# Pixel-Talk/CanonSwap

Hardware: AMD Instinct MI355X
Metric: frames/sec at 512x512 (generator hot path F->W->T->R->W->G) (higher is better)
Workload: dtype f16; 1 GPU; BASELINE configs[2]: 512x512 video, 64 frames batched per launch on each GPU, steady state over 1280 frames (20 launches per GPU) (256x256 crops in, random-init weights of the real architecture); frames_per_launch_per_gpu=64, frames_total=1280, parallelism=frame-shard x1, identities_resident=1, latency_mode=False, accumulate=fp32, debug_decodes=False

## Files before the change

canonswap_amd/_isa.py:

```python
from __future__ import annotations

import os
import subprocess

from ._build import HALO_NGROUPS, OBJ_DIR


def _disassemble(obj_dir: str, objdump: str, oname: str) -> str:
    obj = os.path.join(obj_dir, oname)
    subprocess.run([objdump, "--offloading", obj], check=True, capture_output=True)
    co = obj + ".0.hipv4-amdgcn-amd-amdhsa--gfx950"
    try:
        return subprocess.run([objdump, "-d", "--no-show-raw-insn", co], check=True, capture_output=True, text=True).stdout
    finally:
        for f in os.listdir(obj_dir):
            if f.startswith(oname + ".0."):
                os.remove(os.path.join(obj_dir, f))


def isa_check(obj_dir: str | None = None) -> dict:
    import re
    obj_dir = obj_dir or OBJ_DIR
    objdump = os.environ.get("LLVM_OBJDUMP", "/opt/rocm/lib/llvm/bin/llvm-objdump")
    if not os.path.exists(objdump):
        raise FileNotFoundError(f"isa_check: {objdump} not found")
    seen = dict(_isa_check_wide(obj_dir, objdump))
    seen.update(_isa_check_lat(obj_dir, objdump))
    for g in range(HALO_NGROUPS):
        txt = _disassemble(obj_dir, objdump, f"conv_halo_g{g}.o")
        for m in re.finditer(r"^[0-9a-f]+ <(_Z16conv_halo_kernelILi\d+ELi\d+ELi(\d+)ELi\d+ELi\d+ELi\d+ELb[01]ELb[01]ELi0EEv10ConvParams)>:\n(.*?)(?=^[0-9a-f]+ <|\Z)",
                             txt, re.S | re.M):
            name, wch, body = m.group(1), int(m.group(2)), m.group(3).split("\n")
            want = f"s_waitcnt vmcnt({3 * wch})"
            kend = max(i for i, l in enumerate(body) if "v_mfma" in l)
            waits = [i for i, l in enumerate(body) if i < kend and l.strip().startswith(want) and "lgkmcnt" not in l]
            if len(waits) < 4:
                raise RuntimeError(f"isa_check: {name}: {len(waits)} x `{want}` in the K loop, expected 4 (one per ring slot)")
            waits = waits[:4]
            loads = [(i, re.search(r"global_load_dwordx4 v\[(\d+):(\d+)\], v\[\d+:\d+\], off", l)) for i, l in enumerate(body)]
            loads = [(i, int(q.group(1))) for i, q in loads if q]
            prime = [r for i, r in loads if i < waits[0]][-4 * wch:]
            if len(prime) != 4 * wch:
                raise RuntimeError(f"isa_check: {name}: the prologue primes {len(prime)} ring registers, expected {4 * wch}")
            for k, w in enumerate(waits):
                slot = prime[k * wch:(k + 1) * wch]
                end = waits[k + 1] if k + 1 < 4 else len(body)
                seg = body[w:end]
                rel = [i for i, r in loads if w < i < end and r in slot]
                if len(rel) < wch:
                    raise RuntimeError(f"isa_check: {name}: ring slot {k} is not reloaded into v{slot} after its wait")
                first_reload = min(rel) - w
                uses = [j for j, l in enumerate(seg[:first_reload]) if "v_mfma" in l and any(f"v[{r}:{r + 3}]" in l for r in slot)]
                if not uses:
                    raise RuntimeError(f"isa_check: {name}: no MFMA reads ring slot {k} (v{slot}) between its wait and its reload")
            tail = "\n".join(body[waits[-1]:])
            if "s_waitcnt vmcnt(0)" not in tail:
                raise RuntimeError(f"isa_check: {name}: the ring is not drained (s_waitcnt vmcnt(0)) before the epilogue")
            seen[name] = len(waits)
    if not seen:
        raise RuntimeError("isa_check: no dynamic-shape conv_halo kernel found in the objects (name mangling changed?)")
    return seen


def _isa_check_lat(obj_dir: str, objdump: str) -> dict:
    import re
    txt = _disassemble(obj_dir, objdump, "conv_lat.o")
    seen = {}
    for m in re.finditer(r"^[0-9a-f]+ <(\S*conv_lat_kernel\S*)>:\n(.*?)(?=^[0-9a-f]+ <|\Z)", txt, re.S | re.M):
        name, body = m.group(1), [l.split("//")[0].strip() for l in m.group(2).split("\n")]
        body = [l for l in body if l]
        mf = [i for i, l in enumerate(body) if l.startswith("v_mfma")]
        if not mf:
            raise RuntimeError(f"isa_check: {name}: no MFMA")
        if any(l.startswith(("s_cbranch", "s_branch")) for l in body[mf[0]:mf[-1]]):
            raise RuntimeError(f"isa_check: {name}: a branch inside the K loop (the walk assumes straight-line code)")
        for i, l in enumerate(body):
            if re.search(r"\bm0\b", l):
                ok = l.startswith("s_mov_b32 m0,") and any(b.startswith("buffer_load") and b.endswith("lds") for b in body[i + 1:i + 3])
                if not ok:
                    raise RuntimeError(f"isa_check: {name}: `{l}` touches m0 outside the hidden LDS-DMA sequence")
        nvm, open_dma, nbar, ndma = 0, [], 0, 0
        for i, l in enumerate(body[:mf[-1] + 1]):
            op = l.split()[0]
            if op.startswith(("global_load", "buffer_load", "global_store", "buffer_store", "scratch_load", "scratch_store")):
                if op.startswith("buffer_load") and l.endswith("lds"):
                    open_dma.append(nvm); ndma += 1
                nvm += 1
            if op == "s_barrier":
                nbar += 1
                w = next((body[j] for j in range(i - 1, max(i - 6, -1), -1) if body[j].startswith("s_waitcnt") and "vmcnt" in body[j]), None)
                if w is None and not open_dma:
                    continue
                if w is None:
                    raise RuntimeError(f"isa_check: {name}: barrier {nbar} of the K loop has no vmcnt wait in front of it")
                n = int(re.search(r"vmcnt\((\d+)\)", w).group(1))
                for idx in open_dma:
                    if nvm - idx - 1 < n:
                        raise RuntimeError(f"isa_check: {name}: `{w}` before barrier {nbar} does not cover a DMA piece issued {nvm - idx - 1} vector-memory instructions earlier")
                open_dma = []
        if open_dma:
            raise RuntimeError(f"isa_check: {name}: {len(open_dma)} DMA pieces are never waited for at a chunk head")
        if len(mf) not in (8 * 6 * 8, 8 * 6 * 16) or ndma != 24:
            raise RuntimeError(f"isa_check: {name}: {len(mf)} MFMAs / {ndma} DMA instructions, expected 384 or 768 / 24")
        seen[name] = len(mf)
    if not seen:
        raise RuntimeError("isa_check: no conv_lat kernel found in conv_lat.o (name mangling changed?)")
    return seen


def _isa_check_wide(obj_dir: str, objdump: str) -> dict:
    seen = _isa_check_ring(obj_dir, objdump, "conv_wide.o", r"\S*conv_wide_kernel\S*", 18 * 64)
    seen.update(_isa_check_ring(obj_dir, objdump, "conv_halo_g1.o", r"_Z16conv_halo_kernelILi32ELi8ELi5ELi2ELi2ELi0ELb1ELb0ELi[789]E\S*", None))
    return seen
# ... 67 lines not shown
```

canonswap_amd/csrc/common.h:

```cpp
#pragma once
#include <hip/hip_runtime.h>
#include <stdint.h>

typedef _Float16 half_t;
typedef _Float16 h8_t __attribute__((ext_vector_type(8)));
typedef _Float16 h4_t __attribute__((ext_vector_type(4)));
typedef float f4_t __attribute__((ext_vector_type(4)));

enum { ACT_NONE = 0, ACT_RELU = 1, ACT_LRELU = 2, ACT_SIGMOID = 3, ACT_GELU = 4 };
enum { MODE_STD = 0, MODE_TBLEND = 1, MODE_SPADE = 2, MODE_PIXSHUF = 3,
       MODE_STDSTAT = 4 };
enum { CFG_128x128 = 0, CFG_128x64 = 1, CFG_256x32 = 2, CFG_256x16 = 3 };
enum { CFG_H_128x128 = 10, CFG_H_128x64 = 11, CFG_H_256x32 = 12, CFG_H_128x32 = 13, CFG_H_128x16 = 14, CFG_H_256x16 = 15,
       CFG_H_SK128x32 = 16 , CFG_H_128x256 = 17,
       CFG_H_128x160 = 18 ,
       CFG_H_256x160 = 19 ,
       CFG_H_256x64 = 20 ,
       CFG_VOL32 = 30 , CFG_WIDE = 31 ,
       CFG_LAT = 32  };

struct TDesc {
    void* p;
    long sN, sD, sH, sW;
};

struct ConvParams {
    const half_t* in;
    const half_t* zero;
    long in_sN, in_sD, in_sH, in_sW;
    int N, D, H, W;
    int inD;
    int Cin;
    int cg, cg_cin;
    long in_sG;
    int nchunks;
    int up_shift;
    int KD, KH, KW, PD, PH, PW;
    const half_t* wgt;
    const long* wofs;
    const int* wslot;
    int Cout_pad;
    int Cout;
    int lgTW, lgTH, lgTD;
    int nTW, nTH, nTD, nTN;
    const float* bias;
    const float* bias2;
    int act0;
    float slope0;
    TDesc res;
    int res_f32;
    int res_shift;
    const float* pixscale;
    int ps_stride;
    TDesc out0;
    int out0_f32;
    const float* s2;
    const float* t2;
    int act1;
    float slope1;
    TDesc out1;
    const float* stats;
    float* stat_out;
    float* sk_out;
    int sk_splits;
    int ragged;
    unsigned mg_ncb, mg_tw, mg_th, mg_td;
    int hilo;
    int xcd_map;
    float* kw_out;
    int ep_general;
// ... 216 lines not shown
```

canonswap_amd/csrc/conv_halo.hip:

```cpp
#include "conv_halo_kernel.h"

#ifndef HALO_GROUP
#define HALO_GROUP (-1)
#endif
#define IN_GROUP(g) (HALO_GROUP == -1 || HALO_GROUP == (g))
#define NOT_MINE (-2)

template <int CK, int WPX, int WCH, int WVP, int WVC, int MODE, bool SK, int STV>
static int launch_halo_cfg(const ConvParams& p, hipStream_t st)
{
    if constexpr (STV != 0) {
        using SS = StaticShape<STV>;
        if (p.KD == SS::KD && p.KH == SS::KH && p.KW == SS::KW && p.lgTW == SS::LW && p.lgTH == SS::LH && p.lgTD == SS::LD &&
            p.nchunks % (CK / 32) == 0)
            return launch_halo_st<CK, WPX, WCH, WVP, WVC, MODE, SK, STV>(p, st);
    }
    if constexpr (WCH == 4 && MODE == MODE_STDSTAT) {
        cs_set_error("conv_halo: the 128x256 statistics tile exists for the static shapes only (%dx%dx%d taps, tile 2^%d x 2^%d x 2^%d)",
                     p.KD, p.KH, p.KW, p.lgTW, p.lgTH, p.lgTD);
        return -1;
    } else {
        return launch_halo_st<CK, WPX, WCH, WVP, WVC, MODE, SK, 0>(p, st);
    }
}

#define HALO_CASE(CFG, WPX, WCH, WVP, WVC, MODE, SK, ST2D, ST3D)                                         \
    if (cfg == CFG && mode == MODE) {                                                                    \
        if (ck == 64) return launch_halo_cfg<64, WPX, WCH, WVP, WVC, MODE, SK, ST2D>(p, st);            \
        if (stv == 1) return launch_halo_cfg<32, WPX, WCH, WVP, WVC, MODE, SK, ST2D>(p, st);            \
        if (stv == 5 && ST3D == 2) return launch_halo_cfg<32, WPX, WCH, WVP, WVC, MODE, SK, (ST3D == 2 ? 5 : 0)>(p, st); \
        return launch_halo_cfg<32, WPX, WCH, WVP, WVC, MODE, SK, ST3D>(p, st);                           \
    }

#define GROUP_FN(g) int launch_conv_halo_g##g(const ConvParams& p, int cfg, int ck, int mode, int stv, hipStream_t st)
GROUP_FN(0); GROUP_FN(1); GROUP_FN(2); GROUP_FN(3); GROUP_FN(4); GROUP_FN(5); GROUP_FN(6); GROUP_FN(7);

#if IN_GROUP(0)
GROUP_FN(0)
{
    (void)stv;
    if (p.KD == 3 && p.KH == 2 && p.KW == 2 && ck == 32 && mode == MODE_STD) {
        if (cfg == CFG_H_256x32) return launch_halo_cfg<32, 4, 2, 4, 1, MODE_STD, false, 12>(p, st);
        if (cfg == CFG_H_128x64) return launch_halo_cfg<32, 4, 2, 2, 2, MODE_STD, false, 13>(p, st);
        if (cfg == CFG_H_128x128 && p.lgTW == 2) return launch_halo_cfg<32, 8, 2, 1, 4, MODE_STD, false, 17>(p, st);
        if (cfg == CFG_H_128x128) return launch_halo_cfg<32, 8, 2, 1, 4, MODE_STD, false, 13>(p, st);
    }
    if (mode == MODE_STD && p.KD == 1 && p.KH == 1 && p.KW == 1) {
        if (cfg == CFG_H_128x128 && ck == 32) return launch_halo_cfg<32, 8, 2, 1, 4, MODE_STD, false, 15>(p, st);
        if (cfg == CFG_H_128x64 && ck == 64) return launch_halo_cfg<64, 4, 2, 2, 2, MODE_STD, false, 15>(p, st);
        if (cfg == CFG_H_128x64 && ck == 32) return launch_halo_cfg<32, 4, 2, 2, 2, MODE_STD, false, 15>(p, st);
        if (cfg == CFG_H_128x32 && ck == 64) return launch_halo_cfg<64, 2, 2, 4, 1, MODE_STD, false, 15>(p, st);
        if (cfg == CFG_H_128x32 && ck == 32) return launch_halo_cfg<32, 2, 2, 4, 1, MODE_STD, false, 15>(p, st);
    }
    return NOT_MINE;
}
#endif

#if IN_GROUP(1)
GROUP_FN(1)
{
    if (cfg == CFG_H_128x128 && mode == MODE_STD && ck == 64 && p.KD == 1 && p.KH <= 2 && p.KW <= 2) {
        if (p.KH == 2 && p.KW == 2) return launch_halo_cfg<64, 8, 2, 1, 4, MODE_STD, false, 10>(p, st);
        if (p.KH == 2) return launch_halo_cfg<64, 8, 2, 1, 4, MODE_STD, false, 11>(p, st);
        if (p.KW == 2) return launch_halo_cfg<64, 8, 2, 1, 4, MODE_STD, false, 14>(p, st);
        return launch_halo_cfg<64, 8, 2, 1, 4, MODE_STD, false, 15>(p, st);
    }
    if (cfg == CFG_H_256x64 && mode == MODE_STD && ck == 32) return launch_halo_cfg<32, 8, 2, 2, 2, MODE_STD, false, 7>(p, st);
    if (cfg == CFG_H_256x64 && ck == 64) {
        if (p.KD != 1 || p.KH != 3 || p.KW != 3 || p.lgTW != 4 || p.lgTH != 4 || p.lgTD != 0) {
            cs_set_error("conv_halo: the 2-D 256x64 tile runs 3x3 convs on 16x16 tiles only");
            return -1;
        }
        if (mode == MODE_STD) return launch_halo_st<64, 8, 2, 2, 2, MODE_STD, false, 16>(p, st);
        if (mode == MODE_STDSTAT) return launch_halo_st<64, 8, 2, 2, 2, MODE_STDSTAT, false, 16>(p, st);
    }
    if (cfg == CFG_H_256x160 && mode == MODE_STD && ck == 32) {
        if (p.KD == 7 && p.lgTW == 2) return launch_halo_cfg<32, 8, 5, 2, 2, MODE_STD, false, 9>(p, st);
        if (p.KD == 7) return launch_halo_cfg<32, 8, 5, 2, 2, MODE_STD, false, 8>(p, st);
        return launch_halo_cfg<32, 8, 5, 2, 2, MODE_STD, false, 7>(p, st);
    }
    if (cfg == CFG_H_128x160 && mode == MODE_STD && ck == 32) {
        if (stv == 4) return launch_halo_cfg<32, 4, 5, 2, 2, MODE_STD, false, 4>(p, st);
        if (stv == 6) return launch_halo_cfg<32, 4, 5, 2, 2, MODE_STD, false, 6>(p, st);
        return launch_halo_cfg<32, 4, 5, 2, 2, MODE_STD, false, 2>(p, st);
    }
    return NOT_MINE;
}
#endif

#if IN_GROUP(2)
GROUP_FN(2)
{
    HALO_CASE(CFG_H_128x256, 8, 4, 1, 4, MODE_STD, false, 1, 0)
    HALO_CASE(CFG_H_128x256, 8, 4, 1, 4, MODE_TBLEND, false, 1, 0)
// ... 73 lines not shown
```

canonswap_amd/csrc/conv_halo_kernel.h:

```cpp
#pragma once
#include <type_traits>
#include <utility>
#include <cstdlib>
#include "common.h"
#ifdef CS_TIMELINE
#define EP_TL(i) TL_STAMP(i)
#endif
#define EP_POOL_WSH_V EP_POOL_WSH_K
#define EP_POOL_HSH_V EP_POOL_HSH_K
#define EP_SPMUL_V EP_SPMUL_K
#define EP_DUP_V EP_DUP_K
#define EP_MLIN_V EP_MLIN_K
#define EP_O1ONLY_V EP_O1ONLY_K
#define EP_O0_EXTRA_V ep_o0_extra
#include "conv_epilogue.h"

typedef unsigned int u4_t __attribute__((ext_vector_type(4)));
__device__ __forceinline__ unsigned mdiv(unsigned u, unsigned magic) { return magic ? __umulhi(u, magic) : u; }

template <int OFF>
__device__ __forceinline__ void wfrag_load(u4_t& dst, const half_t* ptr)
{
    asm volatile("global_load_dwordx4 %0, %1, off offset:%2" : "=v"(dst) : "v"(ptr), "n"(OFF));
}
template <int N>
__device__ __forceinline__ void wait_vmcnt_le()
{
    asm volatile("s_waitcnt vmcnt(%0)" ::"n"(N) : "memory");
}

#ifdef CS_TIMELINE
extern unsigned long long* g_cs_tl;
extern long g_cs_tl_cap;
#define TL_STAMP(i) do { __builtin_amdgcn_sched_barrier(0); tl_t[i] = __builtin_amdgcn_s_memtime(); __builtin_amdgcn_sched_barrier(0); } while (0)
#else
#define TL_STAMP(i) do { } while (0)
#endif

template <int ST> struct StaticShape { static constexpr int KD = 0, KH = 0, KW = 0, LW = 0, LH = 0, LD = 0; };
template <> struct StaticShape<1> { static constexpr int KD = 1, KH = 3, KW = 3, LW = 4, LH = 3, LD = 0; };
template <> struct StaticShape<2> { static constexpr int KD = 3, KH = 3, KW = 3, LW = 3, LH = 3, LD = 1; };
template <> struct StaticShape<3> { static constexpr int KD = 3, KH = 3, KW = 3, LW = 2, LH = 2, LD = 4; };
template <> struct StaticShape<4> { static constexpr int KD = 7, KH = 7, KW = 1, LW = 3, LH = 3, LD = 1; };
template <> struct StaticShape<5> { static constexpr int KD = 3, KH = 3, KW = 3, LW = 2, LH = 2, LD = 3; };
template <> struct StaticShape<6> { static constexpr int KD = 7, KH = 7, KW = 1, LW = 1, LH = 3, LD = 3; };
template <> struct StaticShape<7> { static constexpr int KD = 3, KH = 3, KW = 3, LW = 3, LH = 3, LD = 2; };
template <> struct StaticShape<8> { static constexpr int KD = 7, KH = 7, KW = 1, LW = 1, LH = 3, LD = 4; };
template <> struct StaticShape<9> { static constexpr int KD = 7, KH = 7, KW = 1, LW = 2, LH = 3, LD = 3; };
template <> struct StaticShape<16> { static constexpr int KD = 1, KH = 3, KW = 3, LW = 4, LH = 4, LD = 0; };
template <> struct StaticShape<12> { static constexpr int KD = 3, KH = 2, KW = 2, LW = 2, LH = 2, LD = 4; };
template <> struct StaticShape<13> { static constexpr int KD = 3, KH = 2, KW = 2, LW = 3, LH = 3, LD = 1; };
template <> struct StaticShape<17> { static constexpr int KD = 3, KH = 2, KW = 2, LW = 2, LH = 2, LD = 3; };
template <> struct StaticShape<10> { static constexpr int KD = 1, KH = 2, KW = 2, LW = 4, LH = 3, LD = 0; };
template <> struct StaticShape<11> { static constexpr int KD = 1, KH = 2, KW = 1, LW = 4, LH = 3, LD = 0; };
template <> struct StaticShape<14> { static constexpr int KD = 1, KH = 1, KW = 2, LW = 4, LH = 3, LD = 0; };
template <> struct StaticShape<15> { static constexpr int KD = 1, KH = 1, KW = 1, LW = 4, LH = 3, LD = 0; };

template <int CK, int WPX, int WCH, int WVP, int ST, int MODE> constexpr int halo_pad()
{
    if (CK == 64 && WCH == 4 && WPX == 8 && ST == 1) return 2;
    if (CK == 32 && WCH == 5 && WPX == 8 && (ST == 7 || ST == 8 || ST == 9)) return 2;
    if (CK == 64 && WCH == 2 && WPX == 8 && WVP == 2 && ST == 16) return 2;
    if (CK == 32 && WCH == 2 && WPX == 8 && ST == 1 && MODE == MODE_SPADE) return 2;
    return 1;
}
template <int ST, int PAD> constexpr int halo_hi()
{
    if (PAD == 2) return ST == 3 ? 16 : (ST == 9 ? 19 : ((ST == 7 || ST == 8) ? 15 : (ST == 16 ? 13 : 8)));
    return ST == 4 ? 18 : ((ST == 3 || ST == 7 || ST == 8 || ST == 9) ? 13 : (ST == 12 ? 9 : 8));
}
template <int ST, int PAD> __host__ __device__ constexpr int halo_lane_pos(int l)
{
    using SS = StaticShape<ST>;
    if (ST == 0 || SS::KW != 3 || SS::LW > 3 || SS::LW < 2) return l;
    if (SS::LW == 2 && PAD == 2) return ((l & 1) << 1) | ((l & 2) << 2) | ((l >> 2) & 1) | ((l & 8) >> 1);
    return ((l & 1) << 1) | ((l & 2) << 1) | ((l >> 2) & 1) | (l & 8);
}

template <class F, int... I> __device__ __forceinline__ void halo_static_for_impl(F&& f, std::integer_sequence<int, I...>) { (f(std::integral_constant<int, I>{}), ...); }
template <int N, class F> __device__ __forceinline__ void halo_static_for(F&& f) { halo_static_for_impl(static_cast<F&&>(f), std::make_integer_sequence<int, N>{}); }

template <int WCH, int PFS, int HI, int ST0>
constexpr int halo_ring_young(int st, int L, int NP, bool dma_cur)
{
    auto dma = [&](int u, bool on) { return (on && u >= ST0 && u < ST0 + HI) ? 1 : 0; };
    auto cur_before = [&](int from_step ) {
        int n = 0;
        for (int u = from_step; u < st; ++u) n += (u >= 1 ? WCH : 0) + dma(u, dma_cur);
        return n;
    };
    if (st >= PFS) {
        const int u0 = st - PFS + 1;
        return dma(u0, dma_cur) + cur_before(u0 + 1);
    }
    const int prime = (PFS - 1 - st) * WCH + cur_before(0);
    int g = 0;
    if (NP % PFS == 0) g = st + NP - PFS + 1;
    else { for (int u = NP - PFS + 1; u <= NP; ++u) if ((u - 1) % PFS == st) g = u; }
    int carried = dma(g, true);
    for (int u = g + 1; u <= NP; ++u) carried += WCH + (u < NP ? dma(u, true) : 0);
    carried += cur_before(0);
    return prime < carried ? prime : carried;
}

template <int ST, int PAD> constexpr int halo_pool_shift(int bit)
{
    for (int b = 0; b < 4; ++b) if (halo_lane_pos<ST, PAD>(1 << b) == (1 << bit)) return 1 << b;
    return 0;
}

template <int WCH, int ST> constexpr bool halo_phase_group() { return !(ST == 0 && WCH >= 4); }

template <int CK, int WPX, int WCH, int WVP, int MODE, bool SK, int ST> constexpr bool halo_pool2d()
{
    using SS = StaticShape<ST>;
    return ST != 0 && !SK && MODE == MODE_STD && CK == 32 && WPX == 8 && WVP == 1 && (WCH == 2 || WCH == 4) && SS::KD == 1 && SS::KH == 3 && SS::KW == 3 &&
           SS::LW == 4 && SS::LH == 3 && SS::LD == 0;
}

template <int CK, int WPX, int WCH, int WVP, int WVC, int MODE, bool DB, bool SK, int ST>
__global__ void __launch_bounds__(256, (WCH == 4 ? 2 : ((WCH == 2 && WPX == 8 && !SK && ST != 0) ? (WVP == 2 ? 2 : 3) : 1))) conv_halo_kernel(const ConvParams p)
{
    using SS = StaticShape<ST>;
    static_assert(ST == 0 || !SK, "static shapes are not combined with split-K");
    constexpr int BM = SK ? WPX * 16 : WPX * 16 * WVP;
    constexpr int BN = WCH * 16 * WVC;
    constexpr int SL = CK / 8;
    constexpr int PAD = halo_pad<CK, WPX, WCH, WVP, ST, MODE>();
    constexpr int SLP = SL + PAD;
    constexpr bool EP_POOLK = ST != 0 && !SK && MODE == MODE_STD && WCH == 2 && SS::KD == 3 && SS::KH == 3 && SS::KW == 3 && (SS::LW == 3 || SS::LW == 2) && SS::LH >= 1;
    constexpr bool EP_POOLK2 = halo_pool2d<CK, WPX, WCH, WVP, MODE, SK, ST>();
    constexpr bool XSK = ST == 1 && !SK && MODE == MODE_STD && CK == 64 && WCH == 4 && WPX == 8 && WVP == 1;
    constexpr bool EP_SPMUL_K = ST == 1 && !SK && MODE == MODE_STD && CK == 64 && WCH == 4 && WPX == 8 && WVP == 1;
    constexpr bool EP_O1ONLY_K = ST == 16 && !SK && MODE == MODE_STD;
    constexpr bool EP_MLIN_K = ST == 15 && !SK && MODE == MODE_STD;
    constexpr bool EP_DUP_K = (ST == 11 || ST == 14 || ST == 15) && !SK && MODE == MODE_STD && WCH == 2 && WPX == 8;
    constexpr int EP_POOL_WSH_K = EP_POOLK ? halo_pool_shift<ST, PAD>(0) : (EP_POOLK2 ? 1 : 0);
    constexpr int EP_POOL_HSH_K = EP_POOLK ? halo_pool_shift<ST, PAD>(SS::LW) : 0;
    constexpr int VS = SLP * 16;
    constexpr int HI = halo_hi<ST, PAD>();
    constexpr int KH32 = CK / 32;
    constexpr int PFD = 4;
    constexpr int SKS = SK ? 4 : 1;
    static_assert(WVP * WVC == 4, "4 waves per workgroup");
    static_assert(!SK || (WVC == 1 && WPX == 8), "split-K variants: every wave covers all 128 positions");

    extern __shared__ __attribute__((aligned(16))) unsigned char smem[];
#ifdef CS_TIMELINE
    unsigned long long tl_t[8] = {0, 0, 0, 0, 0, 0, 0, 0};
    const unsigned long long tl_real0 = __builtin_amdgcn_s_memrealtime();
    TL_STAMP(0);
#endif

    const int tid = threadIdx.x, lane = tid & 63;
    const int wave = __builtin_amdgcn_readfirstlane(tid >> 6);
    constexpr bool PHK = halo_phase_group<WCH, ST>();
    const int phz = (PHK && p.nphase) ? (int)blockIdx.z : 0;
    const int PHv = (PHK && p.nphase) ? p.ph_PH[phz] : p.PH, PWv = (PHK && p.nphase) ? p.ph_PW[phz] : p.PW;
    const unsigned ep_o0_extra = (PHK && p.nphase) ? p.ph_ooff[phz] : 0u;
    const int wpx = SK ? 0 : wave % WVP, wch = SK ? 0 : wave / WVP;
    const int l15 = lane & 15, l4 = lane >> 4;
    const int l15p = halo_lane_pos<ST, PAD>(l15);
    constexpr int EP_PAIR = ep_pair_of(MODE, WCH);

    constexpr bool ASMRK = DB && !SK && CK == 32 && WCH == 5 && WPX == 8 && WVP == 2 && (ST == 7 || ST == 8 || ST == 9) && MODE == MODE_STD;
    u4_t wr_p[ASMRK ? 3 : 1][ASMRK ? WCH : 1];
    unsigned poffb[ASMRK ? HI : 1];
    __amdgpu_buffer_rsrc_t rsrc_p;
    int gbuf = 0;
    bool staged = false;
    const bool persist = ASMRK && p.persist_total > 0;
    int p_base = 0, p_cnt = 0, p_j = 0, p_i = 0, p_per = 1;
    if (persist) {
        const int total = p.persist_total, G = (int)gridDim.x;
// ... 750 lines not shown
        if (!(poolk || poolk2) || p.res.p || p.out1.p || p.pixscale || p.stat_out || p.out0_f32 || !p.out0.p || p.sk_out || p.ep_general || (p.H & 1) || (p.W & 1) ||
            p.Cout % 8 || p.Cout != p.Cout_pad || (1 << lgS_of(p)) != BM || ((unsigned long long)p.out0.p & 15ull) ||
            ((p.out0.sN | p.out0.sD | p.out0.sH | p.out0.sW) & 7)) {
            cs_set_error("conv_halo: pool_hw (AvgPool(1,2,2) in the epilogue) needs a static 3x3x3 tile of 8 or 4 columns with two channel fragments per wave or a 2-D 16x8 tile with 32-channel chunks, fp16 out0 only, every packed channel real");
            return -1;
        }
    }
    if (p.spmul) {
        if (MODE != MODE_STD || SK || !p.res.p || p.res_f32 || !p.stats || p.out1.p || p.pixscale || p.stat_out || p.pool_hw || p.sk_out || p.kw_out ||
            (1 << lgS_of(p)) != BM) {
            cs_set_error("conv_halo: spmul (out0 = act0(IN(res) (1 + conv))) is a mode-STD epilogue with an fp16 res, stats, one output and tiles within one sample");
            return -1;
        }
    }
    if (p.xs_w) {
        constexpr bool xsk = ST == 1 && !SK && MODE == MODE_STD && CK == 64 && WCH == 4 && WPX == 8 && WVP == 1;
        if (!xsk || !p.spmul || p.out0.p || p.Cout != 256 || p.Cout_pad != 256 || p.xs_cout < 4 || p.xs_cout > 64 || p.xs_cout % 4 || !p.xs_out.p || p.act0 != ACT_NONE ||
            p.lgTW != 4 || p.lgTH != 3 || ((unsigned long long)p.res.p & 15ull) || ((p.res.sN | p.res.sH | p.res.sW) & 7) || ((unsigned long long)p.xs_w & 15ull) ||
            ((unsigned long long)p.xs_out.p & 7ull) || ((p.xs_out.sN | p.xs_out.sH | p.xs_out.sW) & 3) ||
            (p.xs_res.p && (((unsigned long long)p.xs_res.p & 7ull) || ((p.xs_res.sN | p.xs_res.sH | p.xs_res.sW) & 3)))) {
            cs_set_error("conv_halo: xs_w (conv_s inside the spmul epilogue) needs the 128 x 256 tile kernel, 256 modulated channels, no out0, at most 64 shortcut channels");
            return -1;
        }
    }
    if (p.kw_out) {
        constexpr bool kwsum = !SK && MODE == MODE_STD && WCH == 5 && WPX == 8 && WVP == 2 && (ST == 8 || ST == 9);
        if (!kwsum || p.Cout_pad != 160 || p.lgTH != 3 || !((p.lgTW == 1 && p.lgTD == 4) || (p.lgTW == 2 && p.lgTD == 3)) || p.sk_out || p.W % (1 << p.lgTW) ||
            p.nTN != p.N) {
            cs_set_error("conv_halo: kw_out is the mask conv's epilogue (7x7x1 taps, 160 packed channels, 2x8x16 or 4x8x8 tiles of one sample)");
            return -1;
        }
    }
    const int lgS = p.lgTW + p.lgTH + p.lgTD;
    if ((1 << lgS) > BM) { cs_set_error("conv_halo: spatial tile exceeds BM"); return -1; }
    if (MODE == MODE_SPADE && (1 << lgS) != BM) { cs_set_error("conv_halo: SPADE launches must tile within one sample"); return -1; }
    if (MODE == MODE_SPADE && p.res_f32) { cs_set_error("conv_halo: the tensor a SPADE launch modulates is fp16"); return -1; }
    if (p.ragged) {
        constexpr bool ragk = (CK == 32) && (WPX == 8) && (ST == 7 || ST == 8 || ST == 9) && MODE == MODE_STD;
        if (!ragk || SK || p.Cin % 32 != 16 || p.sk_out || p.hilo || p.cg > 0) {
            cs_set_error("conv_halo: paired-tap weights (ragged) need the 256-position 32-channel static kernels and Cin %% 32 == 16");
            return -1;
        }
    }
    if (p.wslot && (1 << lgS) != BM) { cs_set_error("conv_halo: per-sample weight sets need tiles within one sample"); return -1; }
    if (p.cg > 0 && CK != 32 && (!(ST == 15 || (ST == 0 && WCH != 4)) || (p.cg & 1) || (p.in_sG & 63) || p.KD * p.KH * p.KW != 1)) {
        cs_set_error("conv_halo: grouped input channels run 32-channel chunks (64-channel chunks: 1x1 convs with an even number of 32-channel pieces per group)");
        return -1;
    }
    const int TN = BM >> lgS;
    const long HV = (long)TN * ((1 << p.lgTD) + p.KD - 1) * ((1 << p.lgTH) + p.KH - 1) * ((1 << p.lgTW) + p.KW - 1);
    const int nck = (p.Cin + CK - 1) / CK;
    constexpr bool big = (BM == 256 && WCH == 5);
    constexpr bool asmr = WCH == 5 && WPX == 8 && WVP == 2 && (ST == 7 || ST == 8 || ST == 9) && MODE == MODE_STD && !SK;
    const bool db = nck > 1 && (asmr ? 2 * HI * 4096 <= 160 * 1024 : 2 * HV * VS <= (big || (WCH == 4 && PAD == 2) ? 128 : 64) * 1024) && HV * SLP <= 256 * HI;
    size_t lds = (size_t)(db ? 2 : 1) * HV * VS + 16;
    ConvParams kp = p;
    if (asmr && db) {
        lds = (size_t)2 * HI * 4096;
        const long span = (long)(p.inD - 1) * p.in_sD + (long)((p.H - 1) >> p.up_shift) * p.in_sH + (long)((p.W - 1) >> p.up_shift) * p.in_sW + p.Cin + 32;
        if (span >= (1L << 30) || p.cg > 0 || p.hilo || (1 << lgS) != BM) {
            cs_set_error("conv_halo: the 256 x 160 tiles address one sample of the input through a buffer of less than 2^31 bytes (no grouped / split-precision input)");
            return -1;
        }
        kp.in_sample_bytes = (unsigned)(span * 2);
    }
    kp.persist_total = 0;
    if (SK && lds < (size_t)4 * WCH * WPX * 4 * 64 * sizeof(float)) lds = (size_t)4 * WCH * WPX * 4 * 64 * sizeof(float);
    if (p.xs_w && lds < (size_t)32768) lds = 32768;
    if (lds > 160 * 1024) { cs_set_error("conv_halo: halo of %ld voxels does not fit LDS", HV); return -1; }
    dim3 grid((unsigned)(p.nTW * p.nTH * p.nTD * p.nTN), (unsigned)(p.Cout_pad / BN));
    if (p.hilo && (ST == 0 || CK != 32 || nck != 3 || db || p.sk_out)) {
        cs_set_error("conv_halo: the hi/lo split-precision mode needs a static-shape 32-channel kernel with three single-buffered chunks");
        return -1;
    }
    if (p.nphase) {
        if (SK || !halo_phase_group<WCH, ST>() || p.nphase < 1 || p.nphase > 4 || p.sk_out || p.kw_out || p.xs_w || p.persist_total < 0) { cs_set_error("conv_halo: bad grouped launch (%d phases)", p.nphase); return -1; }
        if (p.res.p || p.stat_out || p.pixscale || p.spmul || p.pool_hw) { cs_set_error("conv_halo: a grouped launch carries out0 / out1 only (no res / statistics / pixel scale / spmul / pooling)"); return -1; }
        for (int z = 0; z < p.nphase; ++z)
            if (p.ph_ooff[z] % 8u) { cs_set_error("conv_halo: output offset of phase %d (%u elements) is not a multiple of 8 (16-byte stores)", z, p.ph_ooff[z]); return -1; }
        grid.z = (unsigned)p.nphase;
    }
    if (p.sk_out) {
        if (SK || p.sk_splits < 1 || p.sk_splits > nck || p.xcd_map == 2) { cs_set_error("conv_halo: bad split-K launch (%d splits, %d chunks)", p.sk_splits, nck); return -1; }
        grid.z = (unsigned)p.sk_splits;
    }
    if (p.xcd_map == 2) grid = dim3(grid.x * grid.y, 1, grid.z);
    hipError_t e;
    {
        const unsigned long long umax = (unsigned long long)grid.x * grid.y;
        const unsigned ds[4] = {(unsigned)(p.Cout_pad / BN), (unsigned)p.nTW, (unsigned)p.nTH, (unsigned)p.nTD};
        unsigned mg[4];
        for (int i = 0; i < 4; ++i) {
            if (ds[i] == 0 || umax * ds[i] >= (1ull << 32)) { cs_set_error("conv_halo: launch of %llu workgroups / tile count %u too large", umax, ds[i]); return -1; }
            mg[i] = ds[i] == 1 ? 0u : (unsigned)((1ull << 32) / ds[i]) + 1u;
        }
        kp.mg_ncb = mg[0]; kp.mg_tw = mg[1]; kp.mg_th = mg[2]; kp.mg_td = mg[3];
    }
#ifdef CS_TIMELINE
    kp.tl = g_cs_tl; kp.tl_cap = g_cs_tl_cap;
#endif
    if (asmr && db && p.persist_total != 0 && !p.sk_out && !p.nphase) {
        const unsigned total = grid.x * grid.y;
        kp.persist_total = (int)total;
        grid = dim3(total < 256u ? (total + 7u) & ~7u : 256u, 1);
    }
    if (db) {
        auto k = conv_halo_kernel<CK, WPX, WCH, WVP, WVC, MODE, true, SK, ST>;
// ... 19 lines not shown
```

canonswap_amd/csrc/conv_plan.h:

```cpp
#pragma once
#include "common.h"

struct HaloTile { int BM, BN, wave_px; };
inline HaloTile halo_tile(int hcfg)
{
    switch (hcfg) {
    case CFG_H_128x128: return {128, 128, 64};
    case CFG_H_128x64: return {128, 64, 64};
    case CFG_H_256x32: return {256, 32, 64};
    case CFG_H_128x32: return {128, 32, 32};
    case CFG_H_128x16: return {128, 16, 32};
    case CFG_H_256x16: return {256, 16, 64};
    case CFG_H_SK128x32: return {128, 32, 32};
    case CFG_H_128x256: return {128, 256, 64};
    case CFG_H_128x160: return {128, 160, 64};
    case CFG_H_256x160: return {256, 160, 64};
    case CFG_H_256x64: return {256, 64, 64};
    }
    return {128, 32, 64};
}

inline int ilog2(int v) { int l = 0; while ((1 << l) < v) ++l; return l; }

inline void set_tile(ConvParams& p, int BM, int prefW, int prefH)
{
    int tw = p.W < prefW ? p.W : prefW;
    int th = p.H < prefH ? p.H : prefH;
    while (tw * th > BM) th >>= 1;
    int tdd = BM / (tw * th);
    if (tdd > p.D) tdd = p.D;
    int tn = BM / (tw * th * tdd);
    p.lgTW = ilog2(tw); p.lgTH = ilog2(th); p.lgTD = ilog2(tdd);
    p.nTW = p.W / tw; p.nTH = p.H / th; p.nTD = p.D / tdd; p.nTN = (p.N + tn - 1) / tn;
}

constexpr int HALO_PERSIST = 1;
constexpr int XCD_MAP = 2;

inline int pick_halo_cfg(const ConvParams& p, int mode)
{
    const int Cout_pad = p.Cout_pad;
    if (mode == MODE_PIXSHUF) return CFG_H_256x16;
    if ((mode == MODE_TBLEND || mode == MODE_SPADE || mode == MODE_STD || mode == MODE_STDSTAT) && Cout_pad % 256 == 0 && p.KD == 1 && p.KH == 3 &&
        p.KW == 3 && p.W >= 16 && p.H >= 8 && p.Cin % (mode == MODE_TBLEND ? 32 : 64) == 0 && (long)p.N * p.H * p.W >= 3 * 4096) return CFG_H_128x256;
    if (Cout_pad % 128 == 0) {
        const long tiles = ((long)p.N * p.D * p.H * p.W + 127) / 128;
        const bool k33 = p.KH == 3 && p.KW == 3, k11 = p.KD == 1 && p.KH == 1 && p.KW == 1 && mode == MODE_STD;
        if ((mode == MODE_STD || mode == MODE_STDSTAT) && (k33 || k11) && tiles * (Cout_pad / 128) <= 128)
            return CFG_H_128x64;
        if (k11 && tiles * (Cout_pad / 128) < 256) return CFG_H_128x64;
        return CFG_H_128x128;
    }
    if (Cout_pad == 64 && (mode == MODE_STD || mode == MODE_STDSTAT) && p.KD == 1 && p.KH == 3 && p.KW == 3 && p.Cin % 64 == 0 && p.cg == 0 &&
        p.H % 16 == 0 && p.W % 16 == 0 && p.H >= 128 && !p.sk_out) return CFG_H_256x64;
    if (Cout_pad % 64 == 0) return CFG_H_128x64;
    if (Cout_pad % 32 == 0) return CFG_H_128x32;
    return CFG_H_128x16;
}

struct HaloPlan { int hcfg, ck, stat_nblk; };

inline HaloPlan halo_plan(ConvParams& p, int mode, int hcfg, int prefW, int prefH, bool cg_ck64)
{
    HaloPlan plan;
    plan.hcfg = hcfg >= 0 ? hcfg : pick_halo_cfg(p, mode);
    const HaloTile T = halo_tile(plan.hcfg);
    const bool is3d = p.KD > 1;
    set_tile(p, T.BM, prefW ? prefW : is3d ? 8 : 16, prefH ? prefH : is3d ? 8 : T.BM / 16);
    plan.stat_nblk = p.nTW * p.nTH * p.nTD * (T.BM / T.wave_px);
    const bool spade_ck32 = mode == MODE_SPADE && p.Cout_pad % 256 != 0;
    const bool k11 = p.KD == 1 && p.KH == 1 && p.KW == 1;
    const bool cg64 = cg_ck64 && k11 && p.cg > 0 && !(p.cg & 1) && p.Cin % 64 == 0 && mode == MODE_STD;
    plan.ck = (!is3d && p.Cin % 64 == 0 && (p.cg == 0 || cg64) && !spade_ck32) ? 64 : 32;
    p.xcd_map = XCD_MAP;
    p.persist_total = HALO_PERSIST;
    return plan;
}
```

canonswap_amd/csrc/engine.hip:

```cpp
#include "engine.h"

#include <cstdarg>
#include <initializer_list>

static thread_local char g_err[1024] = "";
void cs_set_error(const char* fmt, ...)
{
    va_list ap;
    va_start(ap, fmt);
    vsnprintf(g_err, sizeof(g_err), fmt, ap);
    va_end(ap);
}
extern "C" const char* cs_last_error(void) { return g_err; }
extern "C" int cs_abi_version(void) { return CS_ABI_VERSION; }

static int need(cs_engine* e, const std::string& n, size_t bytes, const void** out)
{
    const Blob* b = e->find(n);
    if (!b) { cs_set_error("weights: blob '%s' was not uploaded", n.c_str()); return -1; }
    if (bytes && b->bytes != bytes) { cs_set_error("weights: blob '%s' has %zu bytes, expected %zu", n.c_str(), b->bytes, bytes); return -1; }
    *out = b->p;
    return 0;
}

// ... 203 lines not shown
static int run_F(cs_engine* e, int B, const float* img, int* cur, hipStream_t st)
{
    TRY(e->run(1, st, [&] { return launch_conv_first(img, e->first_w, e->first_b, e->f_t0, B, IMG, IMG, st); }, "conv_first"));
    e->flops += 2.0 * 3 * 64 * 9 * (double)B * IMG * IMG;
    ConvCall d0 = mk(e->f_down0, e->f_t0, nhwc(nullptr, 256, 256, 64), B, 1, 256, 256);
    d0.p.act0 = ACT_RELU; wsplit_in(d0, 64);
    d0.p.pool_hw = 1; d0.p.out0 = nhwc(e->f_p0, 128, 128, 128);
    TRY(go(e, d0, st));
    ConvCall d1 = mk(e->f_down1, e->f_p0, nhwc(nullptr, 128, 128, 128), B, 1, 128, 128);
    d1.p.act0 = ACT_RELU; wsplit_in(d1, 128);
    d1.p.pool_hw = 1; d1.p.out0 = nhwc(e->f_p1, 64, 64, 256);
    TRY(go(e, d1, st));
    *cur = 0;
    ConvCall s = mk(e->f_second, e->f_p1, nhwc(nullptr, 64, 64, 256), B, 1, 64, 64);
    s.p.out0 = hwdc2(e->vs[0]); s.p.out0_f32 = 1;
    s.p.out1 = hwdc2(e->va[0]); s.p.s2 = e->f_pre0.s; s.p.t2 = e->f_pre0.t; s.p.act1 = ACT_RELU; wsplit_in(s, 256);
    TRY(go(e, s, st));
    return run_resblocks3d(e, e->f_rb, B, cur, st);
}

static int run_dense_motion(cs_engine* e, int B, const float* feat, const float* kp_d, const float* kp_s, hipStream_t st,
                     const float* warp_in = nullptr, float* warp_o32 = nullptr, half_t* warp_o16 = nullptr, bool want_deform = false,
                     bool shared_feat = false, bool shared_kps = false)
{
    TRY(e->run(1, st, [&] { return launch_dm_compress(feat, e->cmp_w, e->cmp_b, e->dm_comp, shared_feat ? 1 : B, FD, FH, FW, st); }, "dm_compress"));
    e->flops += 2.0 * 32 * 4 * VOX * B;
    TRY(e->run(1, st, [&] { return launch_dm_sparse(e->dm_comp, kp_d, kp_s, e->dm_l[0] + 32, 144, B, FD, FH, FW, st, shared_feat, shared_kps); }, "dm_sparse"));
    static const int cout[5] = {64, 128, 256, 512, 1024};
    static const int skip_off[6] = {32, 64, 128, 256, 512, 0};
    for (int i = 0; i < 5; ++i) {
        const int S = 64 >> i;
        ConvCall c = mk(e->w_enc[i], e->dm_l[i] + skip_off[i], dhwc(nullptr, FD, S, S, DM_LW[i]), B, FD, S, S);
        c.p.act0 = ACT_RELU;
        c.p.out0 = dhwc(e->dm_pre, FD, S, S, cout[i]);
        if (i == 0) c.hcfg = CFG_H_256x64;
        TDesc o = dhwc(e->dm_l[i + 1] + skip_off[i + 1], FD, S / 2, S / 2, DM_LW[i + 1]);
        c.p.pool_hw = 1; c.p.out0 = o;
        TRY(go(e, c, st));
    }
    for (int i = 0; i < 5; ++i) {
        const int lv = 5 - i, S = 64 >> (lv - 1), Si = S / 2;
        ConvCall c = mk(e->w_dec[i], e->dm_l[lv], dhwc(nullptr, FD, Si, Si, DM_LW[lv]), B, FD, S, S, 1);
        c.p.act0 = ACT_RELU;
        c.p.out0 = dhwc(e->dm_l[lv - 1], FD, S, S, DM_LW[lv - 1]);
        if (i >= 3 || (!e->latency_mode && e->knobs.dec_phases_deep)) {
            const int lwo = DM_LW[lv - 1];
            if (!e->knobs.phase_group) {
                for (int ab = 0; ab < 4; ++ab) {
                    const int a = ab >> 1, b = ab & 1;
                    ConvCall q1 = mk(e->w_dec_p[i][ab], e->dm_l[lv], dhwc(nullptr, FD, Si, Si, DM_LW[lv]), B, FD, Si, Si);
                    q1.p.PH = a == 0; q1.p.PW = b == 0;
                    q1.p.act0 = ACT_RELU;
                    q1.p.out0 = td(e->dm_l[lv - 1] + ((long)a * S + b) * lwo, (long)FD * S * S * lwo, (long)S * S * lwo, 2L * S * lwo, 2L * lwo);
                    if (i == 4) { q1.hcfg = CFG_H_256x32; TRY(go(e, q1, st, 4, 4)); }
                    else TRY(go(e, q1, st));
                }
                continue;
            }
            ConvCall q = mk(e->w_dec_p[i][0], e->dm_l[lv], dhwc(nullptr, FD, Si, Si, DM_LW[lv]), B, FD, Si, Si);
            q.p.act0 = ACT_RELU;
            q.p.out0 = td(e->dm_l[lv - 1], (long)FD * S * S * lwo, (long)S * S * lwo, 2L * S * lwo, 2L * lwo);
            q.p.nphase = 4;
            for (int ab = 0; ab < 4; ++ab) {
                const int a = ab >> 1, b = ab & 1;
                q.p.ph_wofs[ab] = (long)(((intptr_t)e->w_dec_p[i][ab].w - (intptr_t)e->w_dec_p[i][0].w) / (intptr_t)sizeof(half_t));
                q.p.ph_ooff[ab] = (unsigned)(((long)a * S + b) * lwo);
                q.p.ph_PH[ab] = a == 0; q.p.ph_PW[ab] = b == 0;
            }
            q.p.PH = 1; q.p.PW = 1;
            static const char* const pn[5] = {"W.dec0.p", "W.dec1.p", "W.dec2.p", "W.dec3.p", "W.dec4.p"};
            q.name = pn[i];
            if (i == 4) { q.hcfg = CFG_H_256x32; TRY(go(e, q, st, 4, 4)); }
            else TRY(go(e, q, st));
            continue;
        }
        if (i == 4) { c.hcfg = CFG_H_256x32; TRY(go(e, c, st, 4, 4)); continue; }
        TRY(go(e, c, st));
    }
    ConvCall t = mk(e->w_tail, e->dm_l[0], dhwc(nullptr, FD, 64, 64, 144), B, FD, 64, 64);
    t.p.act0 = ACT_RELU; t.p.out0 = dhwc(e->dm_pred, FD, 64, 64, 144);
    t.hcfg = CFG_H_256x160;
    TRY(go(e, t, st));
    ConvCall m = mk(e->w_mask, e->dm_pred, dhwc(nullptr, FD, 64, 64, 144), B, FD, 64, 64);
    m.p.kw_out = e->dm_logits;
    m.hcfg = CFG_H_256x160;
    TRY(go(e, m, st, 4, 8));
    if (warp_in && e->knobs.warp_fused) {
        TRY(e->run(2, st, [&] { return launch_dm_softmax_warp(e->dm_logits, e->mask_b, kp_d, kp_s, warp_in, warp_o32, warp_o16, want_deform ? e->dm_deform : nullptr, B, FD, FH, FW, st, shared_feat, shared_kps); },
                   "dm_softmax_warp"));
    } else {
        TRY(e->run(1, st, [&] { return launch_dm_softmax(e->dm_logits, e->mask_b, kp_d, kp_s, e->dm_deform, B, FD, FH, FW, st, shared_kps); }, "dm_softmax"));
        if (warp_in) TRY(e->run(2, st, [&] { return launch_grid_sample(warp_in, e->dm_deform, warp_o32, warp_o16, B, FD, FH, FW, st, shared_feat); }, "grid_sample"));
    }
    if (!e->latency_mode) {
        ConvCall oc = mk(e->w_occ49, e->dm_pred, td(nullptr, (long)FD * 4096 * 144, 0, 64L * 144, 144), B, 1, 64, 64);
        oc.p.cg = 5; oc.p.cg_cin = 144; oc.p.in_sG = 4096L * 144;
        oc.p.out0 = nhwc(e->dm_occpart, 64, 64, 64); oc.p.out0_f32 = 1;
        oc.hcfg = CFG_H_128x64;
        TRY(go(e, oc, st));
        TRY(e->run(1, st, [&] { return launch_occ_finish49(e->dm_occpart, e->occ_b, e->dm_occ, B, 64, 64, st); }, "occ_finish"));
        return 0;
    }
    ConvCall oc = mk(e->w_occ, e->dm_pred, td(nullptr, (long)FD * 4096 * 144, 0, 64L * 144, 144), B, 1, 64, 64);
    oc.p.cg = 5; oc.p.cg_cin = 144; oc.p.in_sG = 4096L * 144;
    oc.p.out0 = nhwc(e->dm_occpart, 64, 64, 16); oc.p.out0_f32 = 1;
    oc.hcfg = e->latency_mode ? CFG_H_128x32 : CFG_H_SK128x32;
    TRY(go(e, oc, st));
    TRY(e->run(1, st, [&] { return launch_occ_finish(e->dm_occpart, e->occ_b, e->dm_occ, B, 64, 64, st); }, "occ_finish"));
    return 0;
}

static int run_warp_out(cs_engine* e, int B, const half_t* vol16, const float* occ, hipStream_t st)
{
    ConvCall t3 = mk(e->w_third, vol16, hwdc2(nullptr), B, 1, 64, 64);
    t3.p.act0 = ACT_LRELU; t3.p.slope0 = 0.01f;
    t3.p.out0 = nhwc(e->w_t3, 64, 64, 256);
    TRY(go(e, t3, st));
    ConvCall f4 = mk(e->w_fourth, e->w_t3, nhwc(nullptr, 64, 64, 256), B, 1, 64, 64);
    f4.p.pixscale = occ;
    f4.p.out0 = nhwc(e->seg16, 64, 64, 256);
    return go(e, f4, st);
}

int t_slots(cs_engine* e, int B, const int* slots, bool* mixed, hipStream_t st)
{
// ... 957 lines not shown
```

canonswap_amd/csrc/knobs.h:

```cpp
#pragma once
#include <cstdlib>

struct Knobs {
    bool vol32;
    bool vol32_xf;
    bool vol32_fused;
    int wide;
    bool warp_fused;
    bool dec_phases_deep;
    bool phase_group;
    bool shortcut_algebra;
    bool shortcut_fuse;
    bool shared_dedup;
    bool amax;
};

struct KnobRow { const char* env; int unset; bool Knobs::*flag; int Knobs::*count; };
constexpr KnobRow KNOB_TABLE[] = {
    {"CANONSWAP_VOL32", 1, &Knobs::vol32, nullptr},
    {"CANONSWAP_VOL32_XF", 1, &Knobs::vol32_xf, nullptr},
    {"CANONSWAP_VOL32_FUSED", 1, &Knobs::vol32_fused, nullptr},
    {"CANONSWAP_WIDE", 1, nullptr, &Knobs::wide},
    {"CANONSWAP_WARP_FUSED", 1, &Knobs::warp_fused, nullptr},
    {"CANONSWAP_DEC_PHASES_DEEP", 1, &Knobs::dec_phases_deep, nullptr},
    {"CANONSWAP_PHASE_GROUP", 1, &Knobs::phase_group, nullptr},
    {"CANONSWAP_SHORTCUT_ALGEBRA", 1, &Knobs::shortcut_algebra, nullptr},
    {"CANONSWAP_SHORTCUT_FUSE", 1, &Knobs::shortcut_fuse, nullptr},
    {"CANONSWAP_SHARED_DEDUP", 1, &Knobs::shared_dedup, nullptr},
    {"CANONSWAP_AMAX", 0, &Knobs::amax, nullptr},
};

inline Knobs knobs_from_env()
{
    Knobs k{};
    for (const KnobRow& r : KNOB_TABLE) {
        const char* s = getenv(r.env);
        const int v = s ? atoi(s) : r.unset;
        if (r.flag) k.*r.flag = v != 0;
        else k.*r.count = v;
    }
    k.vol32_xf = k.vol32_xf && k.vol32;
    k.vol32_fused = k.vol32_fused && k.vol32;
    return k;
}
```

Measured before the change: 541.3 frames/s.

## Add 512x32 and 256x64 halo tiles for batched 3x2x2 decoder up-block convs

Adds two static-shape halo conv tiles (512x32 and 256x64, on 8x8x8 and 8x8x4 position blocks) for the 3x2x2-tap decoder up-block convolutions. In batched mode these tiles are picked when Cout is 32 or 64 and there are enough workgroups. Larger M tiles give more weight reuse per workgroup and fewer launches per phase. The cost is higher register and LDS pressure: occupancy drops to 2 for the new shape, and the 256x64 variant gets a larger double-buffer LDS budget. An ISA check guards against scratch spills.

```diff
diff --git a/canonswap_amd/_isa.py b/canonswap_amd/_isa.py
--- a/canonswap_amd/_isa.py
+++ b/canonswap_amd/_isa.py
@@ -59,6 +59,24 @@
             seen[name] = len(waits)
     if not seen:
         raise RuntimeError("isa_check: no dynamic-shape conv_halo kernel found in the objects (name mangling changed?)")
+    seen.update(_isa_check_dec_tiles(obj_dir, objdump))
+    return seen
+
+
+def _isa_check_dec_tiles(obj_dir: str, objdump: str) -> dict:
+    import re
+    txt = _disassemble(obj_dir, objdump, "conv_halo_g0.o")
+    seen = {}
+    for m in re.finditer(r"^[0-9a-f]+ <(_Z16conv_halo_kernelILi32ELi8ELi2ELi[24]ELi[12]ELi0ELb[01]ELb0ELi1[89]EEv10ConvParams)>:\n(.*?)(?=^[0-9a-f]+ <|\Z)", txt, re.S | re.M):
+        name, body = m.group(1), m.group(2)
+        if re.search(r"^\s*scratch_", body, re.M):
+            raise RuntimeError(f"isa_check: {name} uses scratch")
+        nmfma = len(re.findall(r"^\s*v_mfma", body, re.M))
+        if nmfma == 0 or nmfma % (12 * 16):
+            raise RuntimeError(f"isa_check: {name}: {nmfma} MFMAs, expected a multiple of 12 K-steps x 16")
+        seen[name] = nmfma
+    if len(seen) != 4:
+        raise RuntimeError(f"isa_check: {len(seen)} of the 4 up-block kernels on 128-position waves found in conv_halo_g0.o")
     return seen
 
 
diff --git a/canonswap_amd/csrc/common.h b/canonswap_amd/csrc/common.h
--- a/canonswap_amd/csrc/common.h
+++ b/canonswap_amd/csrc/common.h
@@ -16,6 +16,7 @@
        CFG_H_128x160 = 18 ,
        CFG_H_256x160 = 19 ,
        CFG_H_256x64 = 20 ,
+       CFG_H_512x32 = 21 ,
        CFG_VOL32 = 30 , CFG_WIDE = 31 ,
        CFG_LAT = 32  };
 
diff --git a/canonswap_amd/csrc/conv_halo.hip b/canonswap_amd/csrc/conv_halo.hip
--- a/canonswap_amd/csrc/conv_halo.hip
+++ b/canonswap_amd/csrc/conv_halo.hip
@@ -40,6 +40,16 @@
 {
     (void)stv;
     if (p.KD == 3 && p.KH == 2 && p.KW == 2 && ck == 32 && mode == MODE_STD) {
+        if (cfg == CFG_H_512x32 || cfg == CFG_H_256x64) {
+            const int ld = cfg == CFG_H_512x32 ? 3 : 2;
+            if (p.lgTW != 3 || p.lgTH != 3 || p.lgTD != ld) {
+                cs_set_error("conv_halo: the 3x2x2 convs run the %s tile on 8x8x%d positions only (this launch: 2^%d x 2^%d x 2^%d)",
+                             cfg == CFG_H_512x32 ? "512x32" : "256x64", 1 << ld, p.lgTW, p.lgTH, p.lgTD);
+                return -1;
+            }
+            if (cfg == CFG_H_512x32) return launch_halo_st<32, 8, 2, 4, 1, MODE_STD, false, 18>(p, st);
+            return launch_halo_st<32, 8, 2, 2, 2, MODE_STD, false, 19>(p, st);
+        }
         if (cfg == CFG_H_256x32) return launch_halo_cfg<32, 4, 2, 4, 1, MODE_STD, false, 12>(p, st);
         if (cfg == CFG_H_128x64) return launch_halo_cfg<32, 4, 2, 2, 2, MODE_STD, false, 13>(p, st);
         if (cfg == CFG_H_128x128 && p.lgTW == 2) return launch_halo_cfg<32, 8, 2, 1, 4, MODE_STD, false, 17>(p, st);
diff --git a/canonswap_amd/csrc/conv_halo_kernel.h b/canonswap_amd/csrc/conv_halo_kernel.h
--- a/canonswap_amd/csrc/conv_halo_kernel.h
+++ b/canonswap_amd/csrc/conv_halo_kernel.h
@@ -51,6 +51,8 @@
 template <> struct StaticShape<12> { static constexpr int KD = 3, KH = 2, KW = 2, LW = 2, LH = 2, LD = 4; };
 template <> struct StaticShape<13> { static constexpr int KD = 3, KH = 2, KW = 2, LW = 3, LH = 3, LD = 1; };
 template <> struct StaticShape<17> { static constexpr int KD = 3, KH = 2, KW = 2, LW = 2, LH = 2, LD = 3; };
+template <> struct StaticShape<18> { static constexpr int KD = 3, KH = 2, KW = 2, LW = 3, LH = 3, LD = 3; };
+template <> struct StaticShape<19> { static constexpr int KD = 3, KH = 2, KW = 2, LW = 3, LH = 3, LD = 2; };
 template <> struct StaticShape<10> { static constexpr int KD = 1, KH = 2, KW = 2, LW = 4, LH = 3, LD = 0; };
 template <> struct StaticShape<11> { static constexpr int KD = 1, KH = 2, KW = 1, LW = 4, LH = 3, LD = 0; };
 template <> struct StaticShape<14> { static constexpr int KD = 1, KH = 1, KW = 2, LW = 4, LH = 3, LD = 0; };
@@ -67,7 +69,7 @@
 template <int ST, int PAD> constexpr int halo_hi()
 {
     if (PAD == 2) return ST == 3 ? 16 : (ST == 9 ? 19 : ((ST == 7 || ST == 8) ? 15 : (ST == 16 ? 13 : 8)));
-    return ST == 4 ? 18 : ((ST == 3 || ST == 7 || ST == 8 || ST == 9) ? 13 : (ST == 12 ? 9 : 8));
+    return ST == 4 ? 18 : (ST == 18 ? 16 : ((ST == 3 || ST == 7 || ST == 8 || ST == 9) ? 13 : (ST == 19 ? 10 : (ST == 12 ? 9 : 8))));
 }
 template <int ST, int PAD> __host__ __device__ constexpr int halo_lane_pos(int l)
 {
@@ -119,7 +121,7 @@
 }
 
 template <int CK, int WPX, int WCH, int WVP, int WVC, int MODE, bool DB, bool SK, int ST>
-__global__ void __launch_bounds__(256, (WCH == 4 ? 2 : ((WCH == 2 && WPX == 8 && !SK && ST != 0) ? (WVP == 2 ? 2 : 3) : 1))) conv_halo_kernel(const ConvParams p)
+__global__ void __launch_bounds__(256, (WCH == 4 ? 2 : ((WCH == 2 && WPX == 8 && !SK && ST != 0) ? ((WVP == 2 || ST == 18) ? 2 : 3) : 1))) conv_halo_kernel(const ConvParams p)
 {
     using SS = StaticShape<ST>;
     static_assert(ST == 0 || !SK, "static shapes are not combined with split-K");
@@ -976,7 +978,7 @@
     const int nck = (p.Cin + CK - 1) / CK;
     constexpr bool big = (BM == 256 && WCH == 5);
     constexpr bool asmr = WCH == 5 && WPX == 8 && WVP == 2 && (ST == 7 || ST == 8 || ST == 9) && MODE == MODE_STD && !SK;
-    const bool db = nck > 1 && (asmr ? 2 * HI * 4096 <= 160 * 1024 : 2 * HV * VS <= (big || (WCH == 4 && PAD == 2) ? 128 : 64) * 1024) && HV * SLP <= 256 * HI;
+    const bool db = nck > 1 && (asmr ? 2 * HI * 4096 <= 160 * 1024 : 2 * HV * VS <= (big || (WCH == 4 && PAD == 2) ? 128 : (ST == 19 ? 80 : 64)) * 1024) && HV * SLP <= 256 * HI;
     size_t lds = (size_t)(db ? 2 : 1) * HV * VS + 16;
     ConvParams kp = p;
     if (asmr && db) {
diff --git a/canonswap_amd/csrc/conv_plan.h b/canonswap_amd/csrc/conv_plan.h
--- a/canonswap_amd/csrc/conv_plan.h
+++ b/canonswap_amd/csrc/conv_plan.h
@@ -16,6 +16,7 @@
     case CFG_H_128x160: return {128, 160, 64};
     case CFG_H_256x160: return {256, 160, 64};
     case CFG_H_256x64: return {256, 64, 64};
+    case CFG_H_512x32: return {512, 32, 64};
     }
     return {128, 32, 64};
 }
@@ -58,6 +59,18 @@
     return CFG_H_128x16;
 }
 
+constexpr int DEC_WAVE128_MIN_WGS = 256;
+inline int dec_wave128_cfg(const ConvParams& p, bool batched, bool knob)
+{
+    if (!batched || !knob || p.KD != 3 || p.KH != 2 || p.KW != 2 || (p.Cout_pad != 32 && p.Cout_pad != 64)) return -1;
+    const int hcfg = p.Cout_pad == 32 ? CFG_H_512x32 : CFG_H_256x64;
+    const HaloTile T = halo_tile(hcfg);
+    const int td = T.BM / 64;
+    if (p.W % 8 || p.H % 8 || p.D % td) return -1;
+    const long wgs = (long)p.N * (p.D / td) * (p.H / 8) * (p.W / 8) * (p.nphase > 0 ? p.nphase : 1);
+    return wgs >= DEC_WAVE128_MIN_WGS ? hcfg : -1;
+}
+
 struct HaloPlan { int hcfg, ck, stat_nblk; };
 
 inline HaloPlan halo_plan(ConvParams& p, int mode, int hcfg, int prefW, int prefH, bool cg_ck64)
diff --git a/canonswap_amd/csrc/engine.hip b/canonswap_amd/csrc/engine.hip
--- a/canonswap_amd/csrc/engine.hip
+++ b/canonswap_amd/csrc/engine.hip
@@ -279,7 +279,9 @@
                     q1.p.PH = a == 0; q1.p.PW = b == 0;
                     q1.p.act0 = ACT_RELU;
                     q1.p.out0 = td(e->dm_l[lv - 1] + ((long)a * S + b) * lwo, (long)FD * S * S * lwo, (long)S * S * lwo, 2L * S * lwo, 2L * lwo);
-                    if (i == 4) { q1.hcfg = CFG_H_256x32; TRY(go(e, q1, st, 4, 4)); }
+                    const int w128 = dec_wave128_cfg(q1.p, !e->latency_mode, e->knobs.dec_wave128);
+                    if (w128 >= 0) { q1.hcfg = w128; TRY(go(e, q1, st)); }
+                    else if (i == 4) { q1.hcfg = CFG_H_256x32; TRY(go(e, q1, st, 4, 4)); }
                     else TRY(go(e, q1, st));
                 }
                 continue;
@@ -297,7 +299,9 @@
             q.p.PH = 1; q.p.PW = 1;
             static const char* const pn[5] = {"W.dec0.p", "W.dec1.p", "W.dec2.p", "W.dec3.p", "W.dec4.p"};
             q.name = pn[i];
-            if (i == 4) { q.hcfg = CFG_H_256x32; TRY(go(e, q, st, 4, 4)); }
+            const int w128 = dec_wave128_cfg(q.p, !e->latency_mode, e->knobs.dec_wave128);
+            if (w128 >= 0) { q.hcfg = w128; TRY(go(e, q, st)); }
+            else if (i == 4) { q.hcfg = CFG_H_256x32; TRY(go(e, q, st, 4, 4)); }
             else TRY(go(e, q, st));
             continue;
         }
diff --git a/canonswap_amd/csrc/knobs.h b/canonswap_amd/csrc/knobs.h
--- a/canonswap_amd/csrc/knobs.h
+++ b/canonswap_amd/csrc/knobs.h
@@ -8,6 +8,8 @@
     int wide;
     bool warp_fused;
     bool dec_phases_deep;
+    int dec_phases_form;
+    bool dec_wave128;
     bool phase_group;
     bool shortcut_algebra;
     bool shortcut_fuse;
@@ -22,7 +24,7 @@
     {"CANONSWAP_VOL32_FUSED", 1, &Knobs::vol32_fused, nullptr},
     {"CANONSWAP_WIDE", 1, nullptr, &Knobs::wide},
     {"CANONSWAP_WARP_FUSED", 1, &Knobs::warp_fused, nullptr},
-    {"CANONSWAP_DEC_PHASES_DEEP", 1, &Knobs::dec_phases_deep, nullptr},
+    {"CANONSWAP_DEC_PHASES_DEEP", 1, &Knobs::dec_phases_deep, &Knobs::dec_phases_form},
     {"CANONSWAP_PHASE_GROUP", 1, &Knobs::phase_group, nullptr},
     {"CANONSWAP_SHORTCUT_ALGEBRA", 1, &Knobs::shortcut_algebra, nullptr},
     {"CANONSWAP_SHORTCUT_FUSE", 1, &Knobs::shortcut_fuse, nullptr},
@@ -37,8 +39,9 @@
         const char* s = getenv(r.env);
         const int v = s ? atoi(s) : r.unset;
         if (r.flag) k.*r.flag = v != 0;
-        else k.*r.count = v;
+        if (r.count) k.*r.count = v;
     }
+    k.dec_wave128 = k.dec_phases_form != 2;
     k.vol32_xf = k.vol32_xf && k.vol32;
     k.vol32_fused = k.vol32_fused && k.vol32;
     return k;
```

Measured after the change: 543.7 frames/s, median of 6. Within noise of the previous version (+0.4%).
